# NikNazarov/TorchPIV

Hardware: AMD Instinct MI355X
Metric: image-pairs/sec at 4 MP, wind=64 ov=32 2-pass CWS; % HBM roofline (higher is better)
Workload: dtype u32 exact sums + f64 / f32

## Files before the change

### include/torchpiv_hip.h

```cpp
#ifndef TORCHPIV_HIP_H
#define TORCHPIV_HIP_H

#include <stddef.h>
#include <stdint.h>

#ifdef __cplusplus
extern "C" {
#endif

#define TPIV_VERSION 2

enum tpiv_status {
    TPIV_OK = 0,
    TPIV_EINVAL = 1,
    TPIV_EKEY = 2,
    TPIV_EHIP = 3,
    TPIV_ENOMEM = 4,
    TPIV_EUNSUPPORTED = 5
};

enum tpiv_mode {
    TPIV_MODE_DWS = 1,
    TPIV_MODE_CWS = 2,
    TPIV_MODE_CWS_FAST = 3
// ... 121 lines not shown
                              int n_bufs, size_t slot_bytes, int n_threads);
int tpiv_reader_next(tpiv_reader* reader, int* n_files, int* buf_index, int64_t* sizes);
int tpiv_reader_release(tpiv_reader* reader);
void tpiv_reader_close(tpiv_reader* reader);


int tpiv_plan_set_timing(tpiv_plan* plan, int enable);
int tpiv_plan_get_timing(tpiv_plan* plan, double* avg_ms, int n_slots, int* n_runs);
int tpiv_plan_exact_fallbacks(tpiv_plan* plan, long long* n_windows);
int tpiv_plan_exact_timing(const tpiv_plan* plan, double* ms4);


int tpiv_debug_pass(int mode, int precision, const uint8_t* a_dev, const uint8_t* b_dev, int batch, int H, int W,
                    int ws, int ov, const double* u2_dev, const double* v2_dev, const double* zero_dev,
                    double* u_dev, double* v_dev, uint8_t* invalid_dev,
                    float* win_dev, float* corr_dev, void* work_dev, size_t work_bytes, void* stream);

int tpiv_debug_iter_compact(int mode, const uint8_t* a_dev, const uint8_t* b_dev, int batch, int H, int W,
                            int ws, int ov, const double* u_raw_dev, const double* v_raw_dev, const uint8_t* mask_dev,
                            double val_ratio, int val_win, int precision,
                            double* u_dev, double* v_dev, uint8_t* invalid_dev, double* du_dev, double* dv_dev,
                            void* work_dev, size_t work_bytes, void* stream);

int tpiv_debug_peaks(const float* maps_dev, int n_maps, int ws, int planar, double val_ratio, int val_win,
                     double* u_dev, double* v_dev, uint8_t* invalid_dev,
                     void* work_dev, size_t work_bytes, void* stream);

int tpiv_plan_debug_predict(tpiv_plan* plan, int pass, int batch,
                            const double* u_c_dev, const double* v_c_dev, const uint8_t* invalid_c_dev,
                            double* u0_dev, double* v0_dev, double* u2_dev, double* v2_dev, void* stream);

#ifdef __cplusplus
}
#endif
#endif
```

### torchpiv_amd/_lib.py

```python
from __future__ import annotations

import ctypes as C
import os

_HERE = os.path.dirname(os.path.abspath(__file__))
LIB_PATH = os.environ.get("TPIV_LIB") or os.path.join(_HERE, "libtorchpiv_hip.so")

OK, EINVAL, EKEY, EHIP, ENOMEM, EUNSUPPORTED = 0, 1, 2, 3, 4, 5
MODE_DWS, MODE_CWS, MODE_CWS_FAST = 1, 2, 3
MODES = {"DWS": MODE_DWS, "CWS": MODE_CWS}
ITER_MODES = dict(MODES, CWS_Fast=MODE_CWS_FAST)
PREC_FAST, PREC_REFERENCE, PREC_F64, PREC_EXACT = 0, 1, 2, 3
PRECISIONS = {"fast": PREC_FAST, "reference": PREC_REFERENCE, "f64": PREC_F64, "exact": PREC_EXACT}
PREFILTER_NONE, PREFILTER_MIN, PREFILTER_MEAN = 0, 1, 2
PREFILTERS = {None: PREFILTER_NONE, "min": PREFILTER_MIN, "mean": PREFILTER_MEAN}
ABI_VERSION = 2


class HipError(RuntimeError):
    pass


def _load():
    if not os.path.exists(LIB_PATH):
# ... 45 lines not shown
    "tpiv_postval_compact": (C.c_int, [_f64p, _f64p, _u8p, _vp, _int, _int, _int, _vp, _vp, _f64p, _vp, _vp]),
    "tpiv_finish_fields": (C.c_int, [_f64p, _f64p, _int, _int, _int, C.c_double, C.c_double, _f64p, _f64p, _vp]),
    "tpiv_ensemble_moments": (C.c_int, [_f64p, _f64p, _int, C.c_longlong, _f64p, _vp]),
    "tpiv_bmp_unpack": (C.c_int, [_u8p, _vp, _u8p, _int, _int, _int, _u8p, _vp]),
    "tpiv_bmp_unpack_bg": (C.c_int, [_u8p, _vp, _u8p, _int, _int, _int, _u8p, _u8p, _vp]),
    "tpiv_frame_min": (C.c_int, [_u8p, _int, C.c_longlong, _u8p, _vp]),
    "tpiv_subtract_background": (C.c_int, [_u8p, _int, C.c_longlong, _u8p, _u8p, _vp]),
    "tpiv_prefilter": (C.c_int, [_u8p, _int, _int, _int, _u8p, _int, _int, _int, _u8p, _vp]),
    "tpiv_depth_map": (C.c_int, [_vp, _vp, _int, _int, _int, _u8p, _u8p, _vp]),
    "tpiv_depth_histogram": (C.c_int, [_vp, _int, C.c_longlong, _vp, _vp]),
    "tpiv_equalize_work_bytes": (C.c_size_t, [_int, _int, _int, _int]),
    "tpiv_equalize": (C.c_int, [_u8p, _int, _int, _int, _int, _int, _u8p, _vp, C.c_size_t, _vp]),
    "tpiv_read_files": (C.c_int, [C.POINTER(C.c_char_p), _int, C.c_void_p, C.c_size_t, _int, C.POINTER(C.c_longlong)]),
    "tpiv_reader_open": (C.c_void_p, [C.POINTER(C.c_char_p), C.c_longlong, _int, C.POINTER(C.c_void_p), _int, C.c_size_t, _int]),
    "tpiv_reader_next": (C.c_int, [C.c_void_p, C.POINTER(C.c_int), C.POINTER(C.c_int), C.POINTER(C.c_longlong)]),
    "tpiv_reader_release": (C.c_int, [C.c_void_p]),
    "tpiv_reader_close": (None, [C.c_void_p]),
    "tpiv_plan_set_timing": (C.c_int, [C.c_void_p, _int]),
    "tpiv_plan_get_timing": (C.c_int, [C.c_void_p, C.POINTER(C.c_double), _int, C.POINTER(C.c_int)]),
    "tpiv_plan_debug_predict": (C.c_int, [C.c_void_p, _int, _int, _f64p, _f64p, _u8p, _f64p, _f64p, _f64p,
                                          _f64p, _vp]),
    "tpiv_debug_iter_compact": (C.c_int, [_int, _u8p, _u8p, _int, _int, _int, _int, _int, _f64p, _f64p, _u8p,
                                          _dbl, _int, _int, _f64p, _f64p, _u8p, _f64p, _f64p, _vp, C.c_size_t, _vp]),
    "tpiv_debug_peaks": (C.c_int, [_f32p, _int, _int, _int, _dbl, _int, _f64p, _f64p, _u8p, _vp, C.c_size_t, _vp]),
    "tpiv_debug_pass": (C.c_int, [_int, _int, _u8p, _u8p, _int, _int, _int, _int, _int, _f64p, _f64p, _f64p, _f64p,
                                  _f64p, _u8p, _f32p, _f32p, _vp, C.c_size_t, _vp]),
}

for _name, (_res, _args) in SIGNATURES.items():
    _fn = getattr(lib, _name)
    _fn.restype = _res
    _fn.argtypes = _args


if lib.tpiv_version() != ABI_VERSION:
    raise ImportError(f"{LIB_PATH} has ABI version {lib.tpiv_version()}, this package needs {ABI_VERSION}: rebuild "
                      "(make -C torchpiv_amd/csrc)")


def check(rc: int) -> None:
    if rc == OK:
        return
    msg = lib.tpiv_last_error().decode("utf-8", "replace")
    if rc == EINVAL:
        raise ValueError(msg)
    if rc == EKEY:
# ... 7 lines not shown
```

### torchpiv_amd/csrc/c_api.cpp

```cpp
#include "../../include/torchpiv_hip.h"

#include <hip/hip_runtime.h>

#include <fcntl.h>
#include <sys/stat.h>
#include <unistd.h>

#include <algorithm>
#include <atomic>
#include <condition_variable>
#include <mutex>
#include <cmath>
#include <cstdio>
#include <cstring>
#include <string>
#include <thread>
#include <vector>

#include "piv_kernels.h"

namespace {

thread_local std::string g_err;
#ifdef TPIV_STAMPS
// ... 360 lines not shown
    if (rc) return rc;
    p.peak_raw = static_cast<float*>(work);
    int n_cu;
    rc = n_cu_of_current_device(&n_cu);
    if (rc) return rc;
    HIP_TRY(tpiv::launch_xcorr(p, tpiv::MODE_PASS1, n_cu, (hipStream_t)stream));
    return TPIV_OK;
}

int tpiv_pass1(const uint8_t* a, const uint8_t* b, int batch, int H, int W, int ws, int ov,
               double val_ratio, int val_win, int precision, double* u, double* v, uint8_t* invalid,
               void* work, size_t work_bytes, void* stream) {
    return pass1_impl(a, b, batch, H, W, ws, ov, val_ratio, val_win, precision, u, v, invalid, work, work_bytes,
                      nullptr, nullptr, stream);
}

size_t tpiv_work_bytes(int H, int W, int ws, int ov, int batch) {
    if (ov >= ws || ws > H || ws > W || ws <= 0 || ov < 0 || batch <= 0 || !supported_ws(ws)) return 0;
    int nr, nc;
    field_shape(H, W, ws, ov, &nr, &nc);
    const size_t a = tpiv::peak_raw_bytes(ws, batch, nr * nc, TPIV_PREC_EXACT);
    const size_t a1 = tpiv::peak_raw_bytes(ws, batch, nr * nc, TPIV_PREC_REFERENCE);
    const size_t b = tpiv::peak_raw_bytes(ws, batch, nr * nc, TPIV_PREC_FAST, true);
    return std::max(a, std::max(a1, b));
}

int tpiv_predict(int mode, int batch, int nrc, int ncc, int nrf, int ncf, const double* Ay,
                 const double* Ax, const double* u_c, const double* v_c, const uint8_t* invalid_c,
                 double* work, double* u0, double* v0, double* u2, double* v2, void* stream) {
    if (mode != TPIV_MODE_DWS && mode != TPIV_MODE_CWS) return fail(TPIV_EKEY, "unknown multipass mode");
    if (batch <= 0) return TPIV_OK;
    tpiv::PredictParams q{};
    q.batch = batch;
    q.mode = mode;
    q.nrc = nrc;
    q.ncc = ncc;
    q.nrf = nrf;
    q.ncf = ncf;
    q.Ay = Ay;
    q.Ax = Ax;
    q.u_c = u_c;
    q.v_c = v_c;
    q.val_c = invalid_c;
    q.T = work;
    q.u0 = u0;
    q.v0 = v0;
    q.u2 = u2;
// ... 822 lines not shown
```

### torchpiv_amd/csrc/piv_kernels.h

```cpp
#pragma once
#include <hip/hip_runtime.h>
#include <stdint.h>

namespace tpiv {

enum { MODE_PASS1 = 0, MODE_DWS = 1, MODE_CWS = 2, MODE_CWSF = 3 };

struct PassParams {
    const uint8_t* A;
    const uint8_t* B;
    int batch, H, W;
    int ws, ov, n_rows, n_cols;
    const double* u0;
    const double* v0;
    const double* u2;
    const double* v2;
    const uint8_t* pmask;
    double* u;
    double* v;
    uint8_t* val;
    double* du;
    double* dv;
    double val_ratio;
    int val_win;
    int precision;
    float* dbg_win;
    float* dbg_corr;
    unsigned long long* stamps;
    float* peak_raw;
    unsigned* work_ctr;
    int* slow_list;
    unsigned* slow_count;
    int list_mode;
    uint4* cand;
    int* fb_list;
    unsigned* fb_count;
    float exact_band;
    float exact_band_range;
    hipEvent_t* sub_events;
    unsigned groups_magic, ncols_magic;
    int groups_shift, ncols_shift;
};

constexpr double EXACT_ETA = 6.66;
enum { EXACT_FFT_RADIX2 = 0, EXACT_FFT_MIXED = 1, EXACT_FFT_PLAIN = 2 };
inline double exact_gamma_u(int ws, int kind) {
    double lg = 0.0, rt = 1.0;
    for (int n = 1; n < ws; n *= 2) lg += 1.0;
    while ((rt + 1.0) * (rt + 1.0) <= (double)ws) rt += 1.0;
    rt += 1.0;
    const double f1 = kind == EXACT_FFT_PLAIN ? (ws + 3) * rt : (kind == EXACT_FFT_MIXED ? 64.0 : lg * EXACT_ETA);
    const double i1 = kind == EXACT_FFT_PLAIN ? (double)(ws + 3) : f1;
    return 2.0 * (2.0 * f1 + 1.0) + 5.0 + 2.0 * i1;
}
inline float exact_band_coef(int ws, int kind = EXACT_FFT_RADIX2) {
    return (float)(2.0 * exact_gamma_u(ws, kind) * (1.0 + 1.0 / 16) * 5.9604644775390625e-08);
// ... 74 lines not shown
}
hipError_t launch_equalize(const uint8_t* frames, int n, int H, int W, int tile, int clip_q8, uint8_t* out, uint8_t* luts,
                           hipStream_t stream);

constexpr int OUTLIER_TILE_COLS = 64, OUTLIER_TILE_ROWS = 8;
struct OutlierParams {
    const double* u;
    const double* v;
    const uint8_t* invalid;
    int batch, n_rows, n_cols;
    double threshold, eps;
    int min_neighbours;
    uint8_t* status;
    double* out_u;
    double* out_v;
    int replace;
    uint8_t* invalid_out;
};
hipError_t launch_median_test(const OutlierParams& p, hipStream_t stream);

hipError_t launch_xcorr(const PassParams& p, int mode, int n_cu, hipStream_t stream);
constexpr size_t TILE_CTR_BYTES = 8 * 16 * sizeof(unsigned), TILE_SLOW_HDR_BYTES = 256;
constexpr bool tile_split64(int ws, int mode) { return ws == 64 && mode == MODE_CWS; }
constexpr int tile_occ_c(int ws, int mode) {
    return (ws != 8 && ws != 16 && ws != 32 && ws != 64) ? 0
           : (ws == 16 ? 4 : ((ws == 32 || (ws == 64 && mode != MODE_CWS)) ? 3 : 2));
}
inline int tile_occ(int ws, int mode) { return tile_occ_c(ws, mode); }
#ifdef __HIPCC__
template <int MODE>
__device__ __forceinline__ void pred_half_shift(const PassParams& p, size_t i, double& sx, double& sy) {
    const bool compact = p.pmask != nullptr;
    const double* __restrict__ us = compact ? p.u0 : p.u2;
    const double* __restrict__ vs = compact ? p.v0 : p.v2;
    double u = us[i], v = vs[i];
    if constexpr (MODE == MODE_DWS) {
        const uint8_t* mp = compact ? p.pmask + i : reinterpret_cast<const uint8_t*>(us + i);
        const bool zero = *mp != 0 && compact;
        const double uz = zero ? 0.0 : u, vz = zero ? 0.0 : v;
        sx = compact ? rint(uz / 2) : u;
        sy = compact ? rint(vz / 2) : v;
    } else {
        sx = compact ? u / 2 : u;
        sy = compact ? v / 2 : v;
    }
}
// ... 27 lines not shown
```

### torchpiv_amd/csrc/piv_launch.hip

```cpp
#include <hip/hip_runtime.h>
#include <stdint.h>
#include <stdio.h>
#include <stdlib.h>

#include "piv_kernels.h"

namespace tpiv {

hipError_t launch_xcorr_w8(const PassParams& p, int mode, int n_cu, hipStream_t stream);
hipError_t launch_peak_debug_w8(const PassParams& p, const float* maps, int n_maps, hipStream_t stream);
hipError_t launch_xcorr_ws16(const PassParams& p, int mode, int n_cu, hipStream_t stream);
hipError_t launch_xcorr_ws32(const PassParams& p, int mode, int n_cu, hipStream_t stream);
hipError_t launch_xcorr_ws64(const PassParams& p, int mode, int n_cu, hipStream_t stream);
hipError_t launch_xcorr_big128_pass1(const PassParams& p, int n_cu, hipStream_t stream);
hipError_t launch_peak_debug_ws8(const PassParams& p, const float* maps, int n_maps, int planar, hipStream_t stream);
hipError_t launch_peak_debug_ws16(const PassParams& p, const float* maps, int n_maps, int planar, hipStream_t stream);
hipError_t launch_peak_debug_ws32(const PassParams& p, const float* maps, int n_maps, int planar, hipStream_t stream);
hipError_t launch_peak_debug_ws64(const PassParams& p, const float* maps, int n_maps, int planar, hipStream_t stream);
hipError_t launch_peak_debug_ws128(const PassParams& p, const float* maps, int n_maps, hipStream_t stream);
hipError_t launch_xcorr_generic(const PassParams& p, int mode, int n_cu, void* scratch, hipStream_t stream);
int generic_blocks(int ws, long long items, int n_cu, int elem_bytes);
bool generic_ct_usable(int ws);
int generic_ct_register_size(int ws, int mode);
hipError_t launch_xcorr_f64(const PassParams& p, int n_cu, hipStream_t stream);
// ... 140 lines not shown
    mn = fminf(fminf(red[0], red[1]), fminf(red[2], red[3]));
    for (int i = threadIdx.x; i < nn; i += 256) m[i] = __fadd_rn(__fsub_rn(m[i], mn), 1e-7f);
}

struct ExactLayout {
    size_t cand, list, count, ctr, scratch, total;
};
static ExactLayout exact_layout(int ws, int batch, int n_windows) {
    auto up = [](size_t b) { return (b + 255) / 256 * 256; };
    ExactLayout l;
    l.cand = peak_bytes(batch, n_windows, 1);
    l.list = l.cand + up((size_t)batch * n_windows * sizeof(uint4));
    l.count = l.list + up((size_t)batch * n_windows * sizeof(int));
    l.ctr = l.count + 256;
    l.scratch = l.ctr + WORK_CTR_BYTES;
    l.total = l.scratch;
    if (!tile_size(ws) && ws != 128)
        l.total += (size_t)generic_blocks(ws, (long long)batch * n_windows, 256, 8) * 2 * ws * ws * 2 * 8;
    return l;
}
static bool exact_size(int ws) { return exact_refine_size(ws); }
size_t exact_fallback_count_offset(int batch, int n_windows) { return exact_layout(64, batch, n_windows).count; }

size_t peak_raw_bytes(int ws, int batch, int n_windows, int precision, bool force_generic) {
    if (precision == 3) {
        if (exact_size(ws) && !force_generic) return exact_layout(ws, batch, n_windows).total;
        precision = 1;
    }
    if (tile_size(ws) && !force_generic) {
        if (precision) return peak_bytes(batch, n_windows, 1);
        return work_ctr_offset(batch, n_windows) + WORK_CTR_BYTES +
               (ws == 64 ? TILE_SLOW_HDR_BYTES + (size_t)batch * n_windows * sizeof(int) : 0);
    }
    const int eb = precision ? 8 : 4;
    return peak_bytes(batch, n_windows, precision) +
           (size_t)generic_blocks(ws, (long long)batch * n_windows, 256, eb) * 2 * ws * ws * 2 * eb;
}

static int pass_precision(int precision, int mode, int ws) {
    if (precision == 2) return mode == MODE_PASS1 ? 1 : 0;
    if (precision == 3) return mode == MODE_PASS1 ? (exact_size(ws) ? 3 : 1) : 0;
    return precision;
}

const char* xcorr_kernel_name(int ws, int mode, int precision, char* buf, int len) {
    precision = pass_precision(precision, mode, ws);
    if (precision == 3 && mode == MODE_PASS1) {
        if (ws == 128) snprintf(buf, len, "xcorr_big128_cand_kernel");
        else if (tile_size(ws)) snprintf(buf, len, "xcorr_tile_cand_kernel<%d>", ws);
        else if (generic_ct_usable(ws)) snprintf(buf, len, "xcorr_generic_ct_kernel<0, %d> (cand)", generic_ct_register_size(ws, mode));
        else snprintf(buf, len, "xcorr_generic_kernel<0, float> (cand)");
    } else if (precision && mode == MODE_PASS1) {
        if (ws == 64 || ws == 128) snprintf(buf, len, "xcorr_f64_split_kernel<%d>", ws);
        else if (tile_size(ws)) snprintf(buf, len, "xcorr_f64_tile_kernel<%d>", ws);
        else snprintf(buf, len, "xcorr_generic_kernel<0, double>");
// ... 68 lines not shown
            if (e != hipSuccess) return e;
        }
        mark(0);
        p.dbg_win = p.dbg_corr = q.dbg_win = q.dbg_corr = nullptr;
        e = launch_exact_refine(p, n_cu, stream);
        if (e != hipSuccess) return e;
        mark(1);
        if (tile_size(p.ws) || p.ws == 128) {
            e = launch_xcorr_f64_list(p, n_cu, stream);
        } else {
            q.precision = 1;
            q.cand = nullptr;
            e = launch_xcorr_generic(q, MODE_PASS1, 256, gscratch, stream);
        }
        mark(2);
    } else if (f64) {
        e = (tile_size(p.ws) || p.ws == 128) ? launch_xcorr_f64(p, n_cu, stream) : generic();
    } else if (tile_size(p.ws)) {
        p.work_ctr = reinterpret_cast<unsigned*>(reinterpret_cast<char*>(p.peak_raw) +
                                                 work_ctr_offset(p.batch, p.n_rows * p.n_cols));
        p.list_mode = 0;
        p.slow_list = nullptr;
        p.slow_count = nullptr;
        const bool split = tile_split64(p.ws, mode) && p.precision == 0;
        if (split) {
            p.slow_count = reinterpret_cast<unsigned*>(reinterpret_cast<char*>(p.work_ctr) + WORK_CTR_BYTES);
            p.slow_list = reinterpret_cast<int*>(reinterpret_cast<char*>(p.slow_count) + TILE_SLOW_HDR_BYTES);
        }
        e = hipMemsetAsync(p.work_ctr, 0, WORK_CTR_BYTES + (split ? TILE_SLOW_HDR_BYTES : 0), stream);
        if (e != hipSuccess) return e;
        switch (p.ws) {
            case 8: e = launch_xcorr_w8(p, mode, n_cu, stream); break;
            case 16: e = launch_xcorr_ws16(p, mode, n_cu, stream); break;
            case 32: e = launch_xcorr_ws32(p, mode, n_cu, stream); break;
            default: e = launch_xcorr_ws64(p, mode, n_cu, stream); break;
        }
    } else if (p.ws == 128 && mode == MODE_PASS1) {
        e = launch_xcorr_big128_pass1(p, n_cu, stream);
    } else {
        e = generic();
    }
    if (e != hipSuccess) return e;
    const size_t total = (size_t)p.batch * p.n_rows * p.n_cols;
    size_t blocks = (total + 255) / 256;
    if (blocks > (size_t)n_cu * 32) blocks = (size_t)n_cu * 32;
    if (f64) hipLaunchKernelGGL(finalize_kernel<true>, dim3((unsigned)blocks), dim3(256), 0, stream, p, mode);
// ... 85 lines not shown
```

### torchpiv_amd/csrc/xcorr_tile.hpp

```cpp
#pragma once
#include <hip/hip_runtime.h>
#include <stdint.h>

#include "fft_inreg.hpp"
#include "piv_kernels.h"

namespace tpiv {

template <int WS, bool PLANAR_ = false>
struct TileGeo {
    static constexpr int WPW = 64 / WS;
    static constexpr int TS = WS > 32 ? 32 : WS;
    static constexpr int PITCH = TS + 1;
    static constexpr int NT = 64 / TS;
    static constexpr int TILE = TS * PITCH;
    static constexpr bool PLANAR = PLANAR_;
    static constexpr int HROWS = WS / 2 + 1;
    static constexpr int HTILE = HROWS * PITCH;
    static constexpr int LDS_FLOATS = NT * TILE * (PLANAR ? 1 : 2);
    static constexpr int MAP_PITCH = WS + 1;
    static constexpr int NDW = WS / 4;
};

template <int CTRL>
// ... 499 lines not shown
    }
    qload = 0;
    return 3;
}

__device__ __forceinline__ int clamp_i(int v, int lo, int hi) { return v < lo ? lo : (v > hi ? hi : v); }

__device__ __forceinline__ int classify_row32(int q, int used, int loaded, int HW, int& qload) {
    const int lim = HW - loaded;
    const bool inside = (unsigned)q <= (unsigned)lim;
    const bool before = q + used - 1 <= 0;
    const bool behind = q >= HW - 1;
    qload = inside ? q : (behind && !before ? lim : 0);
    return inside ? 0 : (before ? 1 : (behind ? 2 : 3));
}

template <int N>
__device__ __forceinline__ void fix_row(uint32_t (&d)[N], int cls) {
    const uint32_t px = (cls == 1 ? (d[0] & 0xffu) : (d[N - 1] >> 24)) * 0x01010101u;
#pragma unroll
    for (int i = 0; i < N; ++i) d[i] = cls != 0 ? px : d[i];
}

template <int WS, int MODE, bool FAST = false>
__device__ __forceinline__ void issue_rows(const PassParams& p, const ItemGeom& g, int r, float vx, float vy,
                                           RawRows<WS, MODE>& raw, const CoopOff<WS>& coff) {
    const int HW = p.H * p.W;
    const uint8_t* __restrict__ fa = p.A + (size_t)g.pair * HW;
    const uint8_t* __restrict__ fb = p.B + (size_t)g.pair * HW;
    const long long base = (long long)(g.y0 + r) * p.W + g.x0;
    if constexpr (MODE == MODE_PASS1) {
        load_dwords<WS / 4>(fa + base, raw.a);
        load_dwords<WS / 4>(fb + base, raw.b);
    } else if constexpr (MODE == MODE_DWS) {
        const long long sh = (long long)vy * p.W + (long long)vx;
        raw.qa = base - sh;
        raw.qb = base + sh;
        long long la, lb;
        const int ca = classify_row(raw.qa, WS, WS, HW, la), cb = classify_row(raw.qb, WS, WS, HW, lb);
        raw.reg = __all(ca != 3 && cb != 3) ? 1 : 0;
        raw.cls = ca | (cb << 2);
        raw.fix = (raw.reg && __any(raw.cls != 0)) ? 1 : 0;
        load_dwords<WS / 4>(fa + (raw.reg ? la : base), raw.a);
        load_dwords<WS / 4>(fb + (raw.reg ? lb : base), raw.b);
    } else {
        const CwsRow c = cws_row(g.y0 + r, vy);
        const float fvx = floorf(vx);
        const int W_ = p.W;
        const int ivx = clamp_i(f2i_sat_t(fvx), -W_, W_);
        const int rlo = -8, rhi = p.H + 7;
        const int dya = clamp_i(c.dya, rlo, rhi), uya = clamp_i(c.uya, rlo, rhi);
        const int dyb = clamp_i(c.dyb, rlo, rhi), uyb = clamp_i(c.uyb, rlo, rhi);
        const int xa = g.x0 - ivx - 1, xb = g.x0 + ivx;
        const int qa0 = dya * W_ + xa, qa1 = uya * W_ + xa;
        const int qb0 = dyb * W_ + xb, qb1 = uyb * W_ + xb;
        using CG = CoopGeo<WS>;
        constexpr int LOADED = CG::LOADED;
        const float gxr = (float)(g.x0 + r);
        const float nxa_r = gxr - vx, nxb_r = gxr + vx;
        const float fxa_r = floorf(nxa_r), fxb_r = floorf(nxb_r);
        const bool col_ok = fxa_r == (float)(g.x0 + r - ivx - 1) && fxb_r == (float)(g.x0 + r + ivx) &&
                            fxa_r != nxa_r && fxb_r != nxb_r;
        bool reg = col_ok && fabsf(vx) < (float)p.W && !(FAST && (c.ydeg_a | c.ydeg_b));
        int cls = 0;
        auto classify_own = [&]() TPIV_LAMBDA_INLINE {
            int la0, la1, lb0, lb1;
            const int c0 = classify_row32(qa0, WS + 1, LOADED, HW, la0), c1 = classify_row32(qa1, WS + 1, LOADED, HW, la1);
            const int c2 = classify_row32(qb0, WS + 1, LOADED, HW, lb0), c3 = classify_row32(qb1, WS + 1, LOADED, HW, lb1);
            reg = reg && c0 != 3 && c1 != 3 && c2 != 3 && c3 != 3;
            cls = c0 | (c1 << 2) | (c2 << 4) | (c3 << 6);
        };
        const float gy0f = (float)g.y0;
        const int base_a = clamp_i(f2i_sat_t(floorf(gy0f - vy)), rlo, rhi);
        const int base_b = clamp_i(f2i_sat_t(floorf(gy0f + vy)), rlo, rhi);
        reg = reg && (unsigned)(dya - base_a) <= (unsigned)WS && (unsigned)(uya - base_a) <= (unsigned)WS &&
              (unsigned)(dyb - base_b) <= (unsigned)WS && (unsigned)(uyb - base_b) <= (unsigned)WS;
        const bool inside = base_a >= 0 && base_a + WS < p.H && base_b >= 0 && base_b + WS < p.H &&
                            xa >= 0 && xa + LOADED <= W_ && xb >= 0 && xb + LOADED <= W_;
        const bool all_in = __all(inside);
        if (!all_in) classify_own();
        raw.reg = __all(reg) ? 1 : 0;
        raw.cls = cls;
        raw.fix = (raw.reg && __any(raw.cls != 0)) ? 1 : 0;
        unsigned oa[CG::NCH], ob[CG::NCH];
        if (all_in) {
            const int qa_o = base_a * W_ + xa, qb_o = base_b * W_ + xb;
#pragma unroll
            for (int k = 0; k < CG::NCH; ++k) {
                oa[k] = (unsigned)(qa_o + coff.o[k]);
                ob[k] = (unsigned)(qb_o + coff.o[k]);
            }
        } else {
#pragma unroll
            for (int k = 0; k < CG::NCH; ++k) {
                const int ci = r + WS * k;
                int j, part;
                CG::chunk(ci, j, part);
                int qa_l, qb_l;
                const int ra = clamp_i(base_a + j, rlo, rhi), rb = clamp_i(base_b + j, rlo, rhi);
                classify_row32(ra * W_ + xa, WS + 1, LOADED, HW, qa_l);
                classify_row32(rb * W_ + xb, WS + 1, LOADED, HW, qb_l);
                const bool live = ci < CG::T;
                oa[k] = live ? (unsigned)(qa_l + 16 * part) : 0u;
                ob[k] = live ? (unsigned)(qb_l + 16 * part) : 0u;
            }
        }
#pragma unroll
        for (int k = 0; k < CG::NCH; ++k) {
            load_dwords<4>(fa + oa[k], raw.ca[k]);
            load_dwords<4>(fb + ob[k], raw.cb[k]);
        }
    }
}

__device__ __forceinline__ uint32_t read_unit_x(const uint4* src) {
    uint4 t = *src;
    asm volatile("" : "+v"(t.x), "+v"(t.y), "+v"(t.z), "+v"(t.w));
    return t.x;
}

struct RowSquares {
    unsigned aa, bb;
};
template <int WS, int MODE, int RBH = 1, bool FAST = false, bool SQ = false, int PATH = 0>
__device__ __forceinline__ void convert_rows(const PassParams& p, const ItemGeom& g, int r, int lane, float vx,
                                             float vy, RawRows<WS, MODE>& raw, cf (&x)[WS], float& sa,
                                             float& sb, float* lds, RowSquares* sq = nullptr) {
    const int HW = p.H * p.W;
    const uint8_t* __restrict__ fa = p.A + (size_t)g.pair * HW;
    const uint8_t* __restrict__ fb = p.B + (size_t)g.pair * HW;
    static constexpr int RBL = WS / RBH;
    float* rowbuf = lds + lane * (RBL + 1);
    static constexpr int UNR_DWS = WS <= 16 ? 1 : 4, UNR_CWS = WS <= 16 ? 1 : 2;
    if constexpr (MODE == MODE_PASS1) {
        unsigned ia = 0, ib = 0;
// ... 539 lines not shown
            const unsigned v = (unsigned)__builtin_amdgcn_readfirstlane((int)q_raw);
            q_base = v < (unsigned)(hi - lo) ? lo + (int)v : hi;
            q_left = QCH;
        }
        const int it = q_base + (QCH - q_left);
        --q_left;
        return it;
    };

    auto geom_of = [&](int pos, int w) TPIV_LAMBDA_INLINE {
        ItemGeom g;
        const int item = real_item(pos);
        g.pair = fast_div(item, p.groups_magic, p.groups_shift);
        const int gi = item - g.pair * groups;
        const int win_raw = gi * G::WPW + w;
        g.active = win_raw < N ? 1 : 0;
        g.win = g.active ? win_raw : N - 1;
        const int wrow = fast_div(g.win, p.ncols_magic, p.ncols_shift);
        g.y0 = wrow * st;
        g.x0 = (g.win - wrow * p.n_cols) * st;
        g.fidx = (size_t)g.pair * N + g.win;
        return g;
    };
    auto shift_of = [&](const ItemGeom& g, float& vx, float& vy) TPIV_LAMBDA_INLINE {
        if constexpr (MODE == MODE_PASS1) {
            vx = 0.f;
            vy = 0.f;
        } else {
            if constexpr (MODE == MODE_CWS) {
                pred_half_shift_cws_f32(p, g.fidx, vx, vy);
            } else {
                double sx, sy;
                pred_half_shift<MODE>(p, g.fidx, sx, sy);
                vx = (float)sx;
                vy = (float)sy;
            }
        }
    };

    int item = q_take(q_issue());
    if (item >= hi) return;
    int nitem = q_take(q_issue());
    constexpr bool RECOMPUTE = WS >= 32;
    float vx, vy;
    RawRows<WS, MODE> raw;
    ItemGeom gcur;
    CoopOff<WS> coff;
    if constexpr (MODE == MODE_CWS) coff.init(fresh_lane() % WS, p.W);
    {
        const int l0 = fresh_lane();
        gcur = geom_of(item, l0 / WS);
        shift_of(gcur, vx, vy);
        issue_rows<WS, MODE, FAST>(p, gcur, l0 % WS, vx, vy, raw, coff);
    }

    TPIV_STAMP_DECL
    TPIV_STAMP_START;
    for (int nnitem; item < hi; item = nitem, nitem = nnitem) {
        const unsigned q_raw = q_issue();
#ifdef TPIV_STAMPS
        ++st_iter;
#endif
        const int lane = fresh_lane();
        const int w = lane / WS;
        const int r = lane % WS;
        const ItemGeom g = RECOMPUTE ? geom_of(item, w) : gcur;
        const bool active = g.active != 0;
        const size_t fidx = g.fidx;
        const int nit = nitem < hi ? nitem : item;
        const ItemGeom gnext = geom_of(nit, w);
        float nvx, nvy;
        shift_of(gnext, nvx, nvy);

        if constexpr (ROLE == 1) {
            if (!raw.reg) {
                if (lane == 0) p.slow_list[atomicAdd(p.slow_count, 1u)] = item;
                nnitem = q_take(q_raw);
                issue_rows<WS, MODE, FAST>(p, gnext, r, nvx, nvy, raw, coff);
                vx = nvx;
                vy = nvy;
                if constexpr (!RECOMPUTE) gcur = gnext;
                continue;
            }
        }
        cf x[WS];
        float sa, sb;
        constexpr int NBS = WS >= 32 ? G::WPW : 1;
        int band_s[NBS];
        TPIV_STAMP(0);
        RowSquares sq;
        convert_rows<WS, MODE, RBH, FAST, CAND, ROLE == 1 ? 1 : 0>(p, g, r, lane, vx, vy, raw, x, sa, sb, tile, &sq);
        TPIV_STAMP(1);
        if constexpr (WS >= 64) nnitem = q_take(q_raw);
        if constexpr (WS <= 32) issue_rows<WS, MODE, FAST>(p, gnext, r, nvx, nvy, raw, coff);

        if (p.dbg_win != nullptr && active) {
            int rr = r;
            asm volatile("" : "+v"(rr));
            float* d = p.dbg_win + fidx * 2 * WS * WS + rr * WS;
#pragma unroll
            for (int k = 0; k < WS; ++k) {
                d[k] = x[k].x;
                d[WS * WS + k] = x[k].y;
            }
        }

        bool dead = false;
        float end_scale = 1.0f;
        constexpr bool FASTN = FAST && MODE != MODE_PASS1;
        constexpr bool NOSWAP = WS == 64 && !(MODE == MODE_DWS && FAST);
        auto up_sign = []() TPIV_LAMBDA_INLINE { return fresh_lane() >= 32 ? 0x80000000u : 0u; };
        auto sflip = [](float v, unsigned sg) TPIV_LAMBDA_INLINE { return __uint_as_float(__float_as_uint(v) ^ sg); };
        if constexpr (!FASTN) {
            sa = grp_sum<WS>(sa);
            sb = grp_sum<WS>(sb);
            const float ma = sa * (1.0f / (WS * WS)), mb = sb * (1.0f / (WS * WS));
            float ka = 1.f, kb = 1.f;
// ... 159 lines not shown
                t[ky] = x[FFT_POS<ky, WS>];
            });
            fft_inreg<WS, -1>(t, tw);
            TPIV_STAMP(7);
            cf hs[WS / 2 + 1], z[WS / 2];
            transpose_half<WS, PLANAR>(t, hs, tile, fresh_lane());
            TPIV_STAMP(8);
            c2r_inreg<WS>(hs, z);
            static_for<0, WS>([&](auto xc) TPIV_LAMBDA_INLINE {
                constexpr int x_ = decltype(xc)::value;
                crow[x_] = (x_ & 1) ? z[FFT_POS<x_ / 2, WS / 2>].y : z[FFT_POS<x_ / 2, WS / 2>].x;
            });
        }
        wave_sync();
        TPIV_STAMP(9);

        auto band_of = [&](int w_) TPIV_LAMBDA_INLINE {
            int b_ = band_s[0];
            static_for<1, NBS>([&](auto wc) TPIV_LAMBDA_INLINE { b_ = w_ == decltype(wc)::value ? band_s[decltype(wc)::value] : b_; });
            return __int_as_float(b_);
        };
        if constexpr (WS > 32) {
            const int lane_p = fresh_lane();
            issue_rows<WS, MODE, FAST>(p, geom_of(nit, lane_p / WS), lane_p % WS, nvx, nvy, raw, coff);
        }
        vx = nvx;
        vy = nvy;
        if constexpr (!RECOMPUTE) gcur = gnext;

        TPIV_STAMP(10);
        if constexpr (RECOMPUTE) {
            const int lane_e = fresh_lane();
            const int w_e = lane_e / WS, r_e = lane_e % WS;
            const int item_e = real_item(item);
            const int pair_e = fast_div(item_e, p.groups_magic, p.groups_shift);
            const int win_raw_e = (item_e - pair_e * groups) * G::WPW + w_e;
            const bool active_e = win_raw_e < N;
            const int win_e = active_e ? win_raw_e : N - 1;
            const size_t fidx_e = (size_t)pair_e * N + win_e;
            if constexpr (CAND) peak_candidates<WS>(p, crow, tile, w_e, r_e, active_e, dead, fidx_e, band_of(w_e));
            else peak_analysis<WS, PLANAR, FASTN>(p, crow, tile, w_e, r_e, active_e, dead, fidx_e, end_scale);
        } else {
            if constexpr (CAND) peak_candidates<WS>(p, crow, tile, w, r, active, dead, fidx, band_of(w));
            else peak_analysis<WS, PLANAR, FASTN>(p, crow, tile, w, r, active, dead, fidx, end_scale);
        }
        wave_sync();
        if constexpr (WS < 64) nnitem = q_take(q_raw);
// ... 42 lines not shown
    return hipGetLastError();
}

template <int WS>
static unsigned tile_grid(PassParams& p, int n_cu) {
    using G = TileGeo<WS>;
    const int N = p.n_rows * p.n_cols;
    const long long groups = (N + G::WPW - 1) / G::WPW;
    const long long items = (long long)p.batch * groups;
    if (items <= 0 || items >= (1ll << 31) - 64) return 0;
    fast_div_setup((unsigned)groups, p.groups_magic, p.groups_shift);
    fast_div_setup((unsigned)p.n_cols, p.ncols_magic, p.ncols_shift);
    const long long cap = (long long)n_cu * 64;
    const long long blocks = items < cap ? items : cap;
    return (unsigned)((blocks + 7) / 8 * 8);
}

template <int WS, int MODE>
static hipError_t launch_tile(const PassParams& p_in, int n_cu, hipStream_t stream) {
    PassParams p = p_in;
    const unsigned blocks = tile_grid<WS>(p, n_cu);
    if (blocks == 0) return hipErrorInvalidValue;
    constexpr int OCC = tile_occ_c(WS, MODE);
    if constexpr (MODE != MODE_PASS1) {
        if (p.precision != 0) {
            hipLaunchKernelGGL((xcorr_tile_kernel<WS, MODE, OCC, false>), dim3(blocks), dim3(64), 0, stream, p);
            return hipGetLastError();
        }
    }
    if constexpr (tile_split64(WS, MODE)) {
        if (p.slow_list != nullptr && p.slow_count != nullptr) {
            hipLaunchKernelGGL((xcorr_tile_fastpath_kernel<WS, MODE>), dim3(blocks), dim3(64), 0, stream, p);
            hipError_t e_ = hipGetLastError();
            if (e_ != hipSuccess) return e_;
            e_ = hipMemsetAsync(p.work_ctr, 0, TILE_CTR_BYTES, stream);
            if (e_ != hipSuccess) return e_;
            PassParams q = p;
            q.list_mode = 1;
            long long blocks2 = (long long)n_cu * 8;
            if (blocks2 > blocks) blocks2 = blocks;
            blocks2 = (blocks2 + 7) / 8 * 8;
            hipLaunchKernelGGL((xcorr_tile_kernel<WS, MODE, OCC, true>), dim3((unsigned)blocks2), dim3(64), 0, stream, q);
            return hipGetLastError();
        }
    }
    hipLaunchKernelGGL((xcorr_tile_kernel<WS, MODE, OCC, true>), dim3(blocks), dim3(64), 0, stream, p);
// ... 24 lines not shown
```

### torchpiv_amd/engine.py

```python
from __future__ import annotations

import ctypes as C

import numpy as np
import torch

from . import _lib
from ._lib import ITER_MODES, MODES, PRECISIONS, check, lib


def _stream() -> int:
    return torch.cuda.current_stream().cuda_stream


def _need_cuda(*tensors):
    for t in tensors:
        if t is not None and not t.is_cuda:
            raise RuntimeError("torchpiv_amd: the HIP path needs tensors on a ROCm device "
                               "(there is no CPU fallback)")


def _frames(a: torch.Tensor, b: torch.Tensor):
    _need_cuda(a, b)
    if a.dtype != torch.uint8 or b.dtype != torch.uint8:
# ... 137 lines not shown
def debug_pass(mode, a, b, ws, ov, u2=None, v2=None, precision="reference"):
    prec = _precision(precision)
    a, b = _frames(a, b)
    B, H, W = a.shape
    nr, nc = field_shape(H, W, ws, ov)
    dev = a.device
    N = nr * nc
    u = torch.empty(B, nr, nc, dtype=torch.float64, device=dev)
    v = torch.empty_like(u)
    inv = torch.empty(B, nr, nc, dtype=torch.uint8, device=dev)
    win = torch.empty(B, N, 2, ws, ws, dtype=torch.float32, device=dev)
    corr = torch.empty(B, N, ws, ws, dtype=torch.float32, device=dev)
    m = 0 if mode in (0, None, "PASS1") else ITER_MODES[mode]
    zero = torch.zeros(B, nr, nc, dtype=torch.float64, device=dev) if m else None
    with torch.cuda.device(dev):
        work, nbytes = _work(H, W, ws, ov, B, dev)
        check(lib.tpiv_debug_pass(m, prec, a.data_ptr(), b.data_ptr(), B, H, W, ws, ov,
                                  u2.contiguous().data_ptr() if u2 is not None else None,
                                  v2.contiguous().data_ptr() if v2 is not None else None,
                                  zero.data_ptr() if zero is not None else None,
                                  u.data_ptr(), v.data_ptr(), inv.data_ptr(), win.data_ptr(),
                                  corr.data_ptr(), work.data_ptr(), nbytes, _stream()))
    return u, v, inv, win, corr


def debug_peaks(maps: torch.Tensor, val_ratio=1.2, val_win=3, planar=False):
    _need_cuda(maps)
    maps = maps.contiguous().float()
    n, ws = maps.shape[0], maps.shape[-1]
    u = torch.empty(n, dtype=torch.float64, device=maps.device)
    v = torch.empty_like(u)
    inv = torch.empty(n, dtype=torch.uint8, device=maps.device)
    work = torch.empty(max(n * 32, 16), dtype=torch.uint8, device=maps.device)
    with torch.cuda.device(maps.device):
        check(lib.tpiv_debug_peaks(maps.data_ptr(), n, ws, int(planar), float(val_ratio), int(val_win),
                                   u.data_ptr(), v.data_ptr(), inv.data_ptr(), work.data_ptr(), n * 32, _stream()))
    return u, v, inv


OUTLIER_DEFAULTS = {"threshold": 2.0, "eps": 0.1, "min_neighbours": 3}


def outlier_arg(outlier):
    if outlier is None:
        return None
    if isinstance(outlier, str):
# ... 590 lines not shown
```

Before: 18530.

## Precompute CWS shift and row-origin plan per window in a prepass kernel

Adds a small prepass kernel that computes each window's CWS predictor shift and checks once whether every row of the window maps to a plain in-bounds load. It stores the shift and the two base offsets as a 16-byte record in the work buffer. The tile kernel then reads this record instead of recomputing the shift and running the per-row classification, and takes a short path when the whole wave is plain. The cost is an extra kernel launch and a per-window record that is written and then read back, and the work buffer grows.

```diff
diff --git a/include/torchpiv_hip.h b/include/torchpiv_hip.h
--- a/include/torchpiv_hip.h
+++ b/include/torchpiv_hip.h
@@ -167,6 +167,8 @@
                             double* u_dev, double* v_dev, uint8_t* invalid_dev, double* du_dev, double* dv_dev,
                             void* work_dev, size_t work_bytes, void* stream);
 
+size_t tpiv_debug_cws_plan_offset(int H, int W, int ws, int ov, int batch);
+
 int tpiv_debug_peaks(const float* maps_dev, int n_maps, int ws, int planar, double val_ratio, int val_win,
                      double* u_dev, double* v_dev, uint8_t* invalid_dev,
                      void* work_dev, size_t work_bytes, void* stream);
diff --git a/torchpiv_amd/_lib.py b/torchpiv_amd/_lib.py
--- a/torchpiv_amd/_lib.py
+++ b/torchpiv_amd/_lib.py
@@ -91,6 +91,7 @@
                                           _f64p, _vp]),
     "tpiv_debug_iter_compact": (C.c_int, [_int, _u8p, _u8p, _int, _int, _int, _int, _int, _f64p, _f64p, _u8p,
                                           _dbl, _int, _int, _f64p, _f64p, _u8p, _f64p, _f64p, _vp, C.c_size_t, _vp]),
+    "tpiv_debug_cws_plan_offset": (C.c_size_t, [_int, _int, _int, _int, _int]),
     "tpiv_debug_peaks": (C.c_int, [_f32p, _int, _int, _int, _dbl, _int, _f64p, _f64p, _u8p, _vp, C.c_size_t, _vp]),
     "tpiv_debug_pass": (C.c_int, [_int, _int, _u8p, _u8p, _int, _int, _int, _int, _int, _f64p, _f64p, _f64p, _f64p,
                                   _f64p, _u8p, _f32p, _f32p, _vp, C.c_size_t, _vp]),
diff --git a/torchpiv_amd/csrc/c_api.cpp b/torchpiv_amd/csrc/c_api.cpp
--- a/torchpiv_amd/csrc/c_api.cpp
+++ b/torchpiv_amd/csrc/c_api.cpp
@@ -406,7 +406,15 @@
     const size_t a = tpiv::peak_raw_bytes(ws, batch, nr * nc, TPIV_PREC_EXACT);
     const size_t a1 = tpiv::peak_raw_bytes(ws, batch, nr * nc, TPIV_PREC_REFERENCE);
     const size_t b = tpiv::peak_raw_bytes(ws, batch, nr * nc, TPIV_PREC_FAST, true);
-    return std::max(a, std::max(a1, b));
+    const size_t c = tpiv::peak_raw_bytes(ws, batch, nr * nc, TPIV_PREC_FAST);
+    return std::max(std::max(a, c), std::max(a1, b));
+}
+
+size_t tpiv_debug_cws_plan_offset(int H, int W, int ws, int ov, int batch) {
+    if (ov >= ws || ws > H || ws > W || ws <= 0 || ov < 0 || batch <= 0 || !supported_ws(ws)) return 0;
+    int nr, nc;
+    field_shape(H, W, ws, ov, &nr, &nc);
+    return tpiv::cws_plan_offset(ws, batch, nr * nc);
 }
 
 int tpiv_predict(int mode, int batch, int nrc, int ncc, int nrf, int ncf, const double* Ay,
diff --git a/torchpiv_amd/csrc/piv_kernels.h b/torchpiv_amd/csrc/piv_kernels.h
--- a/torchpiv_amd/csrc/piv_kernels.h
+++ b/torchpiv_amd/csrc/piv_kernels.h
@@ -32,6 +32,7 @@
     int* slow_list;
     unsigned* slow_count;
     int list_mode;
+    const uint4* cws_plan;
     uint4* cand;
     int* fb_list;
     unsigned* fb_count;
@@ -152,6 +153,8 @@
 hipError_t launch_xcorr(const PassParams& p, int mode, int n_cu, hipStream_t stream);
 constexpr size_t TILE_CTR_BYTES = 8 * 16 * sizeof(unsigned), TILE_SLOW_HDR_BYTES = 256;
 constexpr bool tile_split64(int ws, int mode) { return ws == 64 && mode == MODE_CWS; }
+constexpr bool cws_plan_size(int ws) { return ws == 16 || ws == 32 || ws == 64; }
+size_t cws_plan_offset(int ws, int batch, int n_windows);
 constexpr int tile_occ_c(int ws, int mode) {
     return (ws != 8 && ws != 16 && ws != 32 && ws != 64) ? 0
            : (ws == 16 ? 4 : ((ws == 32 || (ws == 64 && mode != MODE_CWS)) ? 3 : 2));
diff --git a/torchpiv_amd/csrc/piv_launch.hip b/torchpiv_amd/csrc/piv_launch.hip
--- a/torchpiv_amd/csrc/piv_launch.hip
+++ b/torchpiv_amd/csrc/piv_launch.hip
@@ -186,6 +186,14 @@
 static bool exact_size(int ws) { return exact_refine_size(ws); }
 size_t exact_fallback_count_offset(int batch, int n_windows) { return exact_layout(64, batch, n_windows).count; }
 
+static size_t tile_list_end(int ws, int batch, int n_windows) {
+    return work_ctr_offset(batch, n_windows) + WORK_CTR_BYTES +
+           (ws == 64 ? TILE_SLOW_HDR_BYTES + (size_t)batch * n_windows * sizeof(int) : 0);
+}
+size_t cws_plan_offset(int ws, int batch, int n_windows) {
+    return cws_plan_size(ws) ? (tile_list_end(ws, batch, n_windows) + 255) / 256 * 256 : 0;
+}
+
 size_t peak_raw_bytes(int ws, int batch, int n_windows, int precision, bool force_generic) {
     if (precision == 3) {
         if (exact_size(ws) && !force_generic) return exact_layout(ws, batch, n_windows).total;
@@ -193,8 +201,8 @@
     }
     if (tile_size(ws) && !force_generic) {
         if (precision) return peak_bytes(batch, n_windows, 1);
-        return work_ctr_offset(batch, n_windows) + WORK_CTR_BYTES +
-               (ws == 64 ? TILE_SLOW_HDR_BYTES + (size_t)batch * n_windows * sizeof(int) : 0);
+        return cws_plan_size(ws) ? cws_plan_offset(ws, batch, n_windows) + (size_t)batch * n_windows * sizeof(uint4)
+                                 : tile_list_end(ws, batch, n_windows);
     }
     const int eb = precision ? 8 : 4;
     return peak_bytes(batch, n_windows, precision) +
@@ -309,6 +317,10 @@
         p.list_mode = 0;
         p.slow_list = nullptr;
         p.slow_count = nullptr;
+        p.cws_plan = (mode == MODE_CWS && cws_plan_size(p.ws))
+                         ? reinterpret_cast<const uint4*>(reinterpret_cast<char*>(p.peak_raw) +
+                                                          cws_plan_offset(p.ws, p.batch, p.n_rows * p.n_cols))
+                         : nullptr;
         const bool split = tile_split64(p.ws, mode) && p.precision == 0;
         if (split) {
             p.slow_count = reinterpret_cast<unsigned*>(reinterpret_cast<char*>(p.work_ctr) + WORK_CTR_BYTES);
diff --git a/torchpiv_amd/csrc/xcorr_tile.hpp b/torchpiv_amd/csrc/xcorr_tile.hpp
--- a/torchpiv_amd/csrc/xcorr_tile.hpp
+++ b/torchpiv_amd/csrc/xcorr_tile.hpp
@@ -545,9 +545,12 @@
     for (int i = 0; i < N; ++i) d[i] = cls != 0 ? px : d[i];
 }
 
-template <int WS, int MODE, bool FAST = false>
+struct PlanOrigins {
+    int qa, qb;
+};
+template <int WS, int MODE, bool FAST = false, bool PLAN = false>
 __device__ __forceinline__ void issue_rows(const PassParams& p, const ItemGeom& g, int r, float vx, float vy,
-                                           RawRows<WS, MODE>& raw, const CoopOff<WS>& coff) {
+                                           RawRows<WS, MODE>& raw, const CoopOff<WS>& coff, PlanOrigins po = PlanOrigins{}) {
     const int HW = p.H * p.W;
     const uint8_t* __restrict__ fa = p.A + (size_t)g.pair * HW;
     const uint8_t* __restrict__ fb = p.B + (size_t)g.pair * HW;
@@ -567,65 +570,78 @@
         load_dwords<WS / 4>(fa + (raw.reg ? la : base), raw.a);
         load_dwords<WS / 4>(fb + (raw.reg ? lb : base), raw.b);
     } else {
-        const CwsRow c = cws_row(g.y0 + r, vy);
-        const float fvx = floorf(vx);
-        const int W_ = p.W;
-        const int ivx = clamp_i(f2i_sat_t(fvx), -W_, W_);
-        const int rlo = -8, rhi = p.H + 7;
-        const int dya = clamp_i(c.dya, rlo, rhi), uya = clamp_i(c.uya, rlo, rhi);
-        const int dyb = clamp_i(c.dyb, rlo, rhi), uyb = clamp_i(c.uyb, rlo, rhi);
-        const int xa = g.x0 - ivx - 1, xb = g.x0 + ivx;
-        const int qa0 = dya * W_ + xa, qa1 = uya * W_ + xa;
-        const int qb0 = dyb * W_ + xb, qb1 = uyb * W_ + xb;
         using CG = CoopGeo<WS>;
-        constexpr int LOADED = CG::LOADED;
-        const float gxr = (float)(g.x0 + r);
-        const float nxa_r = gxr - vx, nxb_r = gxr + vx;
-        const float fxa_r = floorf(nxa_r), fxb_r = floorf(nxb_r);
-        const bool col_ok = fxa_r == (float)(g.x0 + r - ivx - 1) && fxb_r == (float)(g.x0 + r + ivx) &&
-                            fxa_r != nxa_r && fxb_r != nxb_r;
-        bool reg = col_ok && fabsf(vx) < (float)p.W && !(FAST && (c.ydeg_a | c.ydeg_b));
-        int cls = 0;
-        auto classify_own = [&]() TPIV_LAMBDA_INLINE {
-            int la0, la1, lb0, lb1;
-            const int c0 = classify_row32(qa0, WS + 1, LOADED, HW, la0), c1 = classify_row32(qa1, WS + 1, LOADED, HW, la1);
-            const int c2 = classify_row32(qb0, WS + 1, LOADED, HW, lb0), c3 = classify_row32(qb1, WS + 1, LOADED, HW, lb1);
-            reg = reg && c0 != 3 && c1 != 3 && c2 != 3 && c3 != 3;
-            cls = c0 | (c1 << 2) | (c2 << 4) | (c3 << 6);
-        };
-        const float gy0f = (float)g.y0;
-        const int base_a = clamp_i(f2i_sat_t(floorf(gy0f - vy)), rlo, rhi);
-        const int base_b = clamp_i(f2i_sat_t(floorf(gy0f + vy)), rlo, rhi);
-        reg = reg && (unsigned)(dya - base_a) <= (unsigned)WS && (unsigned)(uya - base_a) <= (unsigned)WS &&
-              (unsigned)(dyb - base_b) <= (unsigned)WS && (unsigned)(uyb - base_b) <= (unsigned)WS;
-        const bool inside = base_a >= 0 && base_a + WS < p.H && base_b >= 0 && base_b + WS < p.H &&
-                            xa >= 0 && xa + LOADED <= W_ && xb >= 0 && xb + LOADED <= W_;
-        const bool all_in = __all(inside);
-        if (!all_in) classify_own();
-        raw.reg = __all(reg) ? 1 : 0;
-        raw.cls = cls;
-        raw.fix = (raw.reg && __any(raw.cls != 0)) ? 1 : 0;
         unsigned oa[CG::NCH], ob[CG::NCH];
-        if (all_in) {
-            const int qa_o = base_a * W_ + xa, qb_o = base_b * W_ + xb;
+        bool plain_wave = false;
+        if constexpr (PLAN) plain_wave = __all(po.qa >= 0) != 0;
+        if (plain_wave) {
 #pragma unroll
             for (int k = 0; k < CG::NCH; ++k) {
-                oa[k] = (unsigned)(qa_o + coff.o[k]);
-                ob[k] = (unsigned)(qb_o + coff.o[k]);
-            }
+                oa[k] = (unsigned)(po.qa + coff.o[k]);
+                ob[k] = (unsigned)(po.qb + coff.o[k]);
+            }
+            raw.reg = 1;
+            raw.cls = 0;
+            raw.fix = 0;
         } else {
-#pragma unroll
-            for (int k = 0; k < CG::NCH; ++k) {
-                const int ci = r + WS * k;
-                int j, part;
-                CG::chunk(ci, j, part);
-                int qa_l, qb_l;
-                const int ra = clamp_i(base_a + j, rlo, rhi), rb = clamp_i(base_b + j, rlo, rhi);
-                classify_row32(ra * W_ + xa, WS + 1, LOADED, HW, qa_l);
-                classify_row32(rb * W_ + xb, WS + 1, LOADED, HW, qb_l);
-                const bool live = ci < CG::T;
-                oa[k] = live ? (unsigned)(qa_l + 16 * part) : 0u;
-                ob[k] = live ? (unsigned)(qb_l + 16 * part) : 0u;
+            const CwsRow c = cws_row(g.y0 + r, vy);
+            const float fvx = floorf(vx);
+            const int W_ = p.W;
+            const int ivx = clamp_i(f2i_sat_t(fvx), -W_, W_);
+            const int rlo = -8, rhi = p.H + 7;
+            const int dya = clamp_i(c.dya, rlo, rhi), uya = clamp_i(c.uya, rlo, rhi);
+            const int dyb = clamp_i(c.dyb, rlo, rhi), uyb = clamp_i(c.uyb, rlo, rhi);
+            const int xa = g.x0 - ivx - 1, xb = g.x0 + ivx;
+            const int qa0 = dya * W_ + xa, qa1 = uya * W_ + xa;
+            const int qb0 = dyb * W_ + xb, qb1 = uyb * W_ + xb;
+            constexpr int LOADED = CG::LOADED;
+            const float gxr = (float)(g.x0 + r);
+            const float nxa_r = gxr - vx, nxb_r = gxr + vx;
+            const float fxa_r = floorf(nxa_r), fxb_r = floorf(nxb_r);
+            const bool col_ok = fxa_r == (float)(g.x0 + r - ivx - 1) && fxb_r == (float)(g.x0 + r + ivx) &&
+                                fxa_r != nxa_r && fxb_r != nxb_r;
+            bool reg = col_ok && fabsf(vx) < (float)p.W && !(FAST && (c.ydeg_a | c.ydeg_b));
+            int cls = 0;
+            auto classify_own = [&]() TPIV_LAMBDA_INLINE {
+                int la0, la1, lb0, lb1;
+                const int c0 = classify_row32(qa0, WS + 1, LOADED, HW, la0), c1 = classify_row32(qa1, WS + 1, LOADED, HW, la1);
+                const int c2 = classify_row32(qb0, WS + 1, LOADED, HW, lb0), c3 = classify_row32(qb1, WS + 1, LOADED, HW, lb1);
+                reg = reg && c0 != 3 && c1 != 3 && c2 != 3 && c3 != 3;
+                cls = c0 | (c1 << 2) | (c2 << 4) | (c3 << 6);
+            };
+            const float gy0f = (float)g.y0;
+            const int base_a = clamp_i(f2i_sat_t(floorf(gy0f - vy)), rlo, rhi);
+            const int base_b = clamp_i(f2i_sat_t(floorf(gy0f + vy)), rlo, rhi);
+            reg = reg && (unsigned)(dya - base_a) <= (unsigned)WS && (unsigned)(uya - base_a) <= (unsigned)WS &&
+                  (unsigned)(dyb - base_b) <= (unsigned)WS && (unsigned)(uyb - base_b) <= (unsigned)WS;
+            const bool inside = base_a >= 0 && base_a + WS < p.H && base_b >= 0 && base_b + WS < p.H &&
+                                xa >= 0 && xa + LOADED <= W_ && xb >= 0 && xb + LOADED <= W_;
+            const bool all_in = __all(inside);
+            if (!all_in) classify_own();
+            raw.reg = __all(reg) ? 1 : 0;
+            raw.cls = cls;
+            raw.fix = (raw.reg && __any(raw.cls != 0)) ? 1 : 0;
+            if (all_in) {
+                const int qa_o = base_a * W_ + xa, qb_o = base_b * W_ + xb;
+#pragma unroll
+                for (int k = 0; k < CG::NCH; ++k) {
+                    oa[k] = (unsigned)(qa_o + coff.o[k]);
+                    ob[k] = (unsigned)(qb_o + coff.o[k]);
+                }
+            } else {
+#pragma unroll
+                for (int k = 0; k < CG::NCH; ++k) {
+                    const int ci = r + WS * k;
+                    int j, part;
+                    CG::chunk(ci, j, part);
+                    int qa_l, qb_l;
+                    const int ra = clamp_i(base_a + j, rlo, rhi), rb = clamp_i(base_b + j, rlo, rhi);
+                    classify_row32(ra * W_ + xa, WS + 1, LOADED, HW, qa_l);
+                    classify_row32(rb * W_ + xb, WS + 1, LOADED, HW, qb_l);
+                    const bool live = ci < CG::T;
+                    oa[k] = live ? (unsigned)(qa_l + 16 * part) : 0u;
+                    ob[k] = live ? (unsigned)(qb_l + 16 * part) : 0u;
+                }
             }
         }
 #pragma unroll
@@ -634,6 +650,54 @@
             load_dwords<4>(fb + ob[k], raw.cb[k]);
         }
     }
+}
+
+template <int WS>
+__global__ __launch_bounds__(256) void cws_plan_kernel(PassParams p, int fast, uint4* __restrict__ out) {
+    const int N = p.n_rows * p.n_cols;
+    const long long i = blockIdx.x * 256ll + threadIdx.x;
+    if (i >= (long long)p.batch * N) return;
+    const int win = (int)(i % N);
+    const int wrow = win / p.n_cols;
+    const int st = p.ws - p.ov;
+    const int y0 = wrow * st, x0 = (win - wrow * p.n_cols) * st;
+    float vx, vy;
+    pred_half_shift_cws_f32(p, (size_t)i, vx, vy);
+    const float fvx = floorf(vx);
+    const int W_ = p.W;
+    const int ivx = clamp_i(f2i_sat_t(fvx), -W_, W_);
+    const int rlo = -8, rhi = p.H + 7;
+    const int xa = x0 - ivx - 1, xb = x0 + ivx;
+    const float gy0f = (float)y0;
+    const int base_a = clamp_i(f2i_sat_t(floorf(gy0f - vy)), rlo, rhi);
+    const int base_b = clamp_i(f2i_sat_t(floorf(gy0f + vy)), rlo, rhi);
+    constexpr int LOADED = CoopGeo<WS>::LOADED;
+    unsigned row_span = 0u, row_gap = 1u, col_bad = 0u;
+#pragma unroll 4
+    for (int r = 0; r < WS; ++r) {
+        const CwsRow c = cws_row(y0 + r, vy);
+        const int dya = min(max(c.dya, rlo), rhi), uya = min(max(c.uya, rlo), rhi);
+        const int dyb = min(max(c.dyb, rlo), rhi), uyb = min(max(c.uyb, rlo), rhi);
+        row_span = max(max(row_span, max((unsigned)(dya - base_a), (unsigned)(uya - base_a))),
+                       max((unsigned)(dyb - base_b), (unsigned)(uyb - base_b)));
+        row_gap = min(row_gap, min((unsigned)(c.uya - c.dya), (unsigned)(c.uyb - c.dyb)));
+        const float gxr = (float)(x0 + r);
+        const float nxa_r = gxr - vx, nxb_r = gxr + vx;
+        const float fxa_r = floorf(nxa_r), fxb_r = floorf(nxb_r);
+        const bool col_ok = (fxa_r == (float)(x0 + r - ivx - 1)) & (fxb_r == (float)(x0 + r + ivx)) &
+                            (fxa_r != nxa_r) & (fxb_r != nxb_r);
+        col_bad |= col_ok ? 0u : 1u;
+    }
+    const bool inside = base_a >= 0 && base_a + WS < p.H && base_b >= 0 && base_b + WS < p.H &&
+                        xa >= 0 && xa + LOADED <= W_ && xb >= 0 && xb + LOADED <= W_;
+    const bool plain = fabsf(vx) < (float)p.W && inside && col_bad == 0u && row_span <= (unsigned)WS &&
+                       !(fast && row_gap == 0u);
+    uint4 rec;
+    rec.x = __float_as_uint(vx);
+    rec.y = __float_as_uint(vy);
+    rec.z = plain ? (unsigned)(base_a * W_ + xa) : ~0u;
+    rec.w = plain ? (unsigned)(base_b * W_ + xb) : ~0u;
+    out[i] = rec;
 }
 
 __device__ __forceinline__ uint32_t read_unit_x(const uint4* src) {
@@ -1219,12 +1283,23 @@
         g.fidx = (size_t)g.pair * N + g.win;
         return g;
     };
-    auto shift_of = [&](const ItemGeom& g, float& vx, float& vy) TPIV_LAMBDA_INLINE {
+    constexpr bool PLAN = MODE == MODE_CWS && cws_plan_size(WS);
+    auto shift_of = [&](const ItemGeom& g, float& vx, float& vy, PlanOrigins& po) TPIV_LAMBDA_INLINE {
         if constexpr (MODE == MODE_PASS1) {
             vx = 0.f;
             vy = 0.f;
         } else {
-            if constexpr (MODE == MODE_CWS) {
+            if constexpr (PLAN) {
+                const uint4 rec = p.cws_plan[g.fidx];
+                vx = __uint_as_float(rec.x);
+                vy = __uint_as_float(rec.y);
+                po.qa = (int)rec.z;
+                po.qb = (int)rec.w;
+                if constexpr (WS == 64) {
+                    po.qa = __builtin_amdgcn_readfirstlane(po.qa);
+                    po.qb = __builtin_amdgcn_readfirstlane(po.qb);
+                }
+            } else if constexpr (MODE == MODE_CWS) {
                 pred_half_shift_cws_f32(p, g.fidx, vx, vy);
             } else {
                 double sx, sy;
@@ -1247,8 +1322,9 @@
     {
         const int l0 = fresh_lane();
         gcur = geom_of(item, l0 / WS);
-        shift_of(gcur, vx, vy);
-        issue_rows<WS, MODE, FAST>(p, gcur, l0 % WS, vx, vy, raw, coff);
+        PlanOrigins po{};
+        shift_of(gcur, vx, vy, po);
+        issue_rows<WS, MODE, FAST, PLAN>(p, gcur, l0 % WS, vx, vy, raw, coff, po);
     }
 
     TPIV_STAMP_DECL
@@ -1267,13 +1343,14 @@
         const int nit = nitem < hi ? nitem : item;
         const ItemGeom gnext = geom_of(nit, w);
         float nvx, nvy;
-        shift_of(gnext, nvx, nvy);
+        PlanOrigins npo{};
+        shift_of(gnext, nvx, nvy, npo);
 
         if constexpr (ROLE == 1) {
             if (!raw.reg) {
                 if (lane == 0) p.slow_list[atomicAdd(p.slow_count, 1u)] = item;
                 nnitem = q_take(q_raw);
-                issue_rows<WS, MODE, FAST>(p, gnext, r, nvx, nvy, raw, coff);
+                issue_rows<WS, MODE, FAST, PLAN>(p, gnext, r, nvx, nvy, raw, coff, npo);
                 vx = nvx;
                 vy = nvy;
                 if constexpr (!RECOMPUTE) gcur = gnext;
@@ -1289,7 +1366,7 @@
         convert_rows<WS, MODE, RBH, FAST, CAND, ROLE == 1 ? 1 : 0>(p, g, r, lane, vx, vy, raw, x, sa, sb, tile, &sq);
         TPIV_STAMP(1);
         if constexpr (WS >= 64) nnitem = q_take(q_raw);
-        if constexpr (WS <= 32) issue_rows<WS, MODE, FAST>(p, gnext, r, nvx, nvy, raw, coff);
+        if constexpr (WS <= 32) issue_rows<WS, MODE, FAST, PLAN>(p, gnext, r, nvx, nvy, raw, coff, npo);
 
         if (p.dbg_win != nullptr && active) {
             int rr = r;
@@ -1495,7 +1572,7 @@
         };
         if constexpr (WS > 32) {
             const int lane_p = fresh_lane();
-            issue_rows<WS, MODE, FAST>(p, geom_of(nit, lane_p / WS), lane_p % WS, nvx, nvy, raw, coff);
+            issue_rows<WS, MODE, FAST, PLAN>(p, geom_of(nit, lane_p / WS), lane_p % WS, nvx, nvy, raw, coff, npo);
         }
         vx = nvx;
         vy = nvy;
@@ -1584,6 +1661,14 @@
     const unsigned blocks = tile_grid<WS>(p, n_cu);
     if (blocks == 0) return hipErrorInvalidValue;
     constexpr int OCC = tile_occ_c(WS, MODE);
+    if constexpr (MODE == MODE_CWS && cws_plan_size(WS)) {
+        if (p.cws_plan == nullptr) return hipErrorInvalidValue;
+        const long long total = (long long)p.batch * p.n_rows * p.n_cols;
+        hipLaunchKernelGGL((cws_plan_kernel<WS>), dim3((unsigned)((total + 255) / 256)), dim3(256), 0, stream, p,
+                           p.precision == 0 ? 1 : 0, const_cast<uint4*>(p.cws_plan));
+        const hipError_t e_ = hipGetLastError();
+        if (e_ != hipSuccess) return e_;
+    }
     if constexpr (MODE != MODE_PASS1) {
         if (p.precision != 0) {
             hipLaunchKernelGGL((xcorr_tile_kernel<WS, MODE, OCC, false>), dim3(blocks), dim3(64), 0, stream, p);
diff --git a/torchpiv_amd/engine.py b/torchpiv_amd/engine.py
--- a/torchpiv_amd/engine.py
+++ b/torchpiv_amd/engine.py
@@ -183,6 +183,37 @@
                                   u.data_ptr(), v.data_ptr(), inv.data_ptr(), win.data_ptr(),
                                   corr.data_ptr(), work.data_ptr(), nbytes, _stream()))
     return u, v, inv, win, corr
+
+
+def debug_cws_plan(a, b, ws, ov, u2, v2, precision="fast", mask=None):
+    prec = _precision(precision)
+    a, b = _frames(a, b)
+    _need_cuda(u2, v2, mask)
+    B, H, W = a.shape
+    nr, nc = field_shape(H, W, ws, ov)
+    dev = a.device
+    off = int(lib.tpiv_debug_cws_plan_offset(H, W, ws, ov, B))
+    if off == 0:
+        raise ValueError(f"no plan records at window size {ws}")
+    u = torch.empty(B, nr, nc, dtype=torch.float64, device=dev)
+    v = torch.empty_like(u)
+    inv = torch.empty(B, nr, nc, dtype=torch.uint8, device=dev)
+    u2, v2 = u2.contiguous(), v2.contiguous()
+    with torch.cuda.device(dev):
+        work, nbytes = _work(H, W, ws, ov, B, dev)
+        if mask is None:
+            zero = torch.zeros_like(u)
+            check(lib.tpiv_iter(ITER_MODES["CWS"], a.data_ptr(), b.data_ptr(), B, H, W, ws, ov, zero.data_ptr(),
+                                zero.data_ptr(), u2.data_ptr(), v2.data_ptr(), 1.2, 3, prec, u.data_ptr(), v.data_ptr(),
+                                inv.data_ptr(), None, None, work.data_ptr(), nbytes, _stream()))
+        else:
+            check(lib.tpiv_debug_iter_compact(ITER_MODES["CWS"], a.data_ptr(), b.data_ptr(), B, H, W, ws, ov, u2.data_ptr(),
+                                              v2.data_ptr(), mask.contiguous().data_ptr(), 1.2, 3, prec, u.data_ptr(),
+                                              v.data_ptr(), inv.data_ptr(), None, None, work.data_ptr(), nbytes, _stream()))
+        rec = work[off:off + 16 * B * nr * nc].clone().view(B, nr, nc, 16)
+    f = rec[..., :8].contiguous().view(torch.float32)
+    q = rec[..., 8:].contiguous().view(torch.int32)
+    return f[..., 0], f[..., 1], q[..., 0], q[..., 1]
 
 
 def debug_peaks(maps: torch.Tensor, val_ratio=1.2, val_win=3, planar=False):
```

Result: no change. 18570 (median of 6 runs) (+0.2%).
